# apache/arrow

Hardware: AMD Instinct MI355X
Metric: filter_take_mrows_per_s (higher is better)
Workload: dtype int64; 1 GPU; Filter+Take int64[1000000000] + validity (10% null), boolean mask 10% true, FilterOptions::DROP; take indices = the mask's row numbers (monotonic; indices_nonzero: uint64 through CallFunction, GetTakeIndices: uint32 in the mirror), no boundscheck; inputs = splitmix64 streams of SURVEY.md 8(d) (seeds 1,2,3); rows=1000000000, selected_rows=99992053, parallelism=single-gpu

## Files before the change

arrow_amd/_lib.py:

```python
from __future__ import annotations

import ctypes as C
import os

_HERE = os.path.dirname(os.path.abspath(__file__))
LIB_PATH = os.path.join(_HERE, "libarrow_amd.so")

ARX_OK = 0
ARX_OUT_OF_MEMORY = -1
ARX_INVALID = -4
ARX_CAPACITY_ERROR = -6
ARX_INDEX_ERROR = -7
ARX_NOT_IMPLEMENTED = -10
ARX_DEVICE_ERROR = -100

ABI_VERSION = 3

FILTER_DROP, FILTER_EMIT_NULL = 0, 1
SORT_ASCENDING, SORT_DESCENDING = 0, 1
NULLS_AT_START, NULLS_AT_END = 0, 1


class ArrowAmdError(Exception):
    """Base class; subclasses mirror pyarrow.lib.ArrowInvalid & friends."""
# ... 61 lines not shown
        ("validity", C.c_void_p),
        ("offsets", C.c_void_p),
        ("data", C.c_void_p),
        ("offset", C.c_int64),
        ("length", C.c_int64),
        ("null_count", C.c_int64),
    ]


_p, _i64, _int, _u64, _u32, _sz = C.c_void_p, C.c_int64, C.c_int, C.c_uint64, C.c_uint32, C.c_size_t
_span = C.POINTER(ArxSpan)
_bspan = C.POINTER(ArxBinarySpan)

SIGNATURES = {
    "arx_last_error": (C.c_char_p, []),
    "arx_abi_version": (_int, []),
    "arx_device_count": (_int, []),
    "arx_set_option": (_int, [C.c_char_p, _i64]),
    "arx_get_counter": (_i64, [C.c_char_p]),
    "arx_filter_workspace_bytes": (_sz, [_i64]),
    "arx_filter_count": (_int, [_span, _int, _p, _sz, C.POINTER(_i64), _p]),
    "arx_filter_count_async": (_int, [_span, _int, _p, _sz, _p]),
    "arx_filter_count_nulls": (_int, [_span, _span, _int, _p, _sz, C.POINTER(_i64), C.POINTER(_i64), _p]),
    "arx_filter_exec": (_int, [_span, _int, _span, _int, _p, _i64, _p, _p, _p]),
    "arx_mask_to_indices": (_int, [_span, _int, _p, _i64, _int, _p, _p, _p]),
    "arx_take_workspace_bytes": (_sz, []),
    "arx_check_index_bounds": (_int, [_span, _int, _u64, _p, _sz, _p]),
    "arx_take": (_int, [_span, _int, _span, _int, _p, _p, _p, _p]),
    "arx_take_rows": (_int, [_span, _i64, _span, _int, _p, _p, _p, _p]),
    "arx_take_bits": (_int, [_span, _span, _int, _p, _p, _p, _p]),
    "arx_binary_take_workspace_bytes": (_sz, [_i64]),
    "arx_binary_take_offsets": (_int, [_bspan, _span, _int, _p, _sz, _p, _p, _p, C.POINTER(_i64), _p]),
    "arx_binary_take_data": (_int, [_bspan, _i64, _p, _sz, _p, _i64, _p, _p]),
    "arx_large_binary_take_workspace_bytes": (_sz, [_i64]),
    "arx_large_binary_take_offsets": (_int, [_bspan, _span, _int, _p, _sz, _p, _p, _p, C.POINTER(_i64), _p]),
    "arx_large_binary_take_data": (_int, [_bspan, _i64, _p, _sz, _p, _i64, _p, _p]),
    "arx_list_take_data": (_int, [_bspan, _int, _i64, _p, _sz, _p, _i64, _p, _p]),
    "arx_large_list_take_data": (_int, [_bspan, _int, _i64, _p, _sz, _p, _i64, _p, _p]),
    "arx_plain_byte_array_offsets": (_int, [_p, _sz, _i64, C.c_int32, _p]),
    "arx_rle_scan_runs": (_int, [_p, _sz, _int, _i64, _u32, _u64, _p, _i64, C.POINTER(_i64), C.POINTER(_i64)]),
    "arx_rle_decode_u32": (_int, [_p, _sz, _p, _i64, _int, _i64, _p, _p]),
    "arx_rle_decode_equals_bitmap": (_int, [_p, _sz, _p, _i64, _int, _i64, _u32, _p, _p]),
    "arx_expand_by_mask": (_int, [_p, _int, _span, _p, _p, _p]),
    "arx_rle_levels_to_bitmap": (_int, [_p, _p, _i64, _p, _p, _p, _p]),
    "arx_rle_scan_runs_equals": (_int, [_p, _sz, _int, _i64, _u32, _u32, _u64, _p, _i64, C.POINTER(_i64), C.POINTER(_i64)]),
    "arx_levels_to_list_workspace_bytes": (_sz, [_i64]),
# ... 191 lines not shown
```

arrow_amd/csrc/plugin/common.inc:

```

std::atomic<int64_t> g_gpu_calls{0};
std::atomic<int64_t> g_stock_calls{0};
std::atomic<int64_t> g_min_rows{1 << 16};
std::atomic<int64_t> g_min_rows_streaming{INT64_MAX};
std::atomic<int64_t> g_filter_morsel_rows{[] {
  const char* env = std::getenv("ARROW_AMD_FILTER_MORSEL_ROWS");
  return env != nullptr ? static_cast<int64_t>(std::strtoll(env, nullptr, 10)) : int64_t(1) << 20;
}()};

std::atomic<bool> g_parquet_pinned_staging{true};
std::atomic<bool> g_parquet_device_levels{true};
std::atomic<int> g_parquet_read_threads{4};
std::atomic<int64_t> g_parquet_read_part_bytes{int64_t(1) << 23};
std::atomic<bool> g_parquet_device_snappy{[] {
  const char* env = std::getenv("ARROW_AMD_PARQUET_DEVICE_SNAPPY");
  return env == nullptr || std::strtoll(env, nullptr, 10) != 0;
}()};
std::atomic<int64_t> g_parquet_device_snappy_pages{0};
std::atomic<bool> g_parquet_device_gzip{true};
std::atomic<int64_t> g_parquet_device_gzip_pages{0};
std::atomic<int64_t> g_parquet_copied_pages{0};

std::atomic<int64_t> g_aggregate_flush_rows{[] {
  const char* env = std::getenv("ARROW_AMD_AGGREGATE_FLUSH_ROWS");
// ... 119 lines not shown
      ptr_ = nullptr;
      size_ = 0;
      const size_t want = std::max<size_t>(bytes + bytes / 4, size_t(1) << 20);
      HIP_RETURN_NOT_OK(hipHostMalloc(&ptr_, want, hipHostMallocDefault));
      size_ = want;
    }
    *out = static_cast<uint8_t*>(ptr_);
    return Status::OK();
  }
  void Trim(size_t keep_at_most) {
    if (size_ > keep_at_most && ptr_ != nullptr) {
      (void)hipHostFree(ptr_);
      ptr_ = nullptr;
      size_ = 0;
    }
  }

 private:
  void* ptr_ = nullptr;
  size_t size_ = 0;
};
thread_local PinnedStaging t_pinned;

enum Slot { kValues = 0, kValidity, kArg2, kArg2Validity, kOutData, kOutValidity, kWs, kCounter, kBinWs, kFlag };

Status Upload(const ArraySpan& a, int byte_width_or_0_for_bool, int data_slot, int validity_slot,
              hipStream_t st, ArxSpan* out) {
  const int64_t o8 = a.offset % 8;
  const int64_t first = a.offset - o8;
  out->offset = o8;
  out->length = a.length;
  out->null_count = a.null_count;
  out->validity = nullptr;
  out->data = nullptr;
  const int64_t span_elems = o8 + a.length;
  if (a.buffers[1].data != nullptr && a.length > 0) {
    const uint8_t* src;
    size_t bytes;
    if (byte_width_or_0_for_bool == 0) {
      src = a.buffers[1].data + first / 8;
      bytes = static_cast<size_t>(arrow::bit_util::BytesForBits(span_elems));
    } else {
      src = a.buffers[1].data + first * byte_width_or_0_for_bool;
      bytes = static_cast<size_t>(span_elems) * byte_width_or_0_for_bool;
    }
    void* d = nullptr;
// ... 66 lines not shown
```

arrow_amd/csrc/plugin/selection.inc:

```
StockKernel g_stock_filter;

arrow::Result<std::unique_ptr<cp::KernelState>> FilterInit(cp::KernelContext* ctx,
                                                           const cp::KernelInitArgs& args) {
  auto state = std::make_unique<ShimState<cp::FilterOptions>>();
  if (g_stock_filter.init) {
    ARROW_ASSIGN_OR_RAISE(state->stock, g_stock_filter.init(ctx, args));
  }
  if (args.options != nullptr) {
    state->options = *static_cast<const cp::FilterOptions*>(args.options);
  }
  return state;
}

Status BooleanTakeOnDevice(const ArxSpan& dv, const ArxSpan& di, int tid, hipStream_t st, ArrayData* out_arr) {
  const int64_t m = di.length;
  const int64_t bytes = ((m + 63) / 64) * 8;
  const bool allocate_validity = dv.null_count != 0 || di.null_count != 0;
  out_arr->length = m;
  out_arr->buffers.resize(2);
  out_arr->buffers[0] = nullptr;
  ARROW_ASSIGN_OR_RAISE(out_arr->buffers[1], AllocDevice(bytes));
  void* d_valid = nullptr;
  void* d_counter = nullptr;
  if (allocate_validity) {
// ... 108 lines not shown
        d_valid = reinterpret_cast<void*>(out_arr->buffers[0]->mutable_address());
      }
      ARROW_RETURN_NOT_OK(FromArx(arx_filter_exec(&dv, w, &dm, null_sel, ws, n,
                                                  reinterpret_cast<void*>(out_arr->buffers[1]->mutable_address()),
                                                  d_valid, st)));
      int64_t selected = 0, set_bits = 0;
      HIP_RETURN_NOT_OK(hipMemcpyAsync(&selected, ws, 8, hipMemcpyDeviceToHost, st));
      if (allocate_validity) {
        void* cws = nullptr;
        ARROW_RETURN_NOT_OK(t_scratch.Get(kCounter, 64, &cws));
        ARROW_RETURN_NOT_OK(FromArx(arx_bitmap_popcount(d_valid, 0, n, cws, 64, &set_bits, st)));
      } else {
        HIP_RETURN_NOT_OK(hipStreamSynchronize(st));
      }
      out_arr->length = selected;
      out_arr->null_count = allocate_validity ? selected - set_bits : 0;
      static_cast<RocmBuffer*>(out_arr->buffers[1].get())->Shrink(selected * w);
      if (allocate_validity) static_cast<RocmBuffer*>(out_arr->buffers[0].get())->Shrink(((selected + 63) / 64) * 8);
      CountGpu(kFnFilter);
      return Status::OK();
    }
    int64_t out_len = 0, out_nulls = 0;
    if (allocate_validity) {
      ARROW_RETURN_NOT_OK(FromArx(arx_filter_count_nulls(&dv, &dm, null_sel, ws, ws_bytes, &out_len, &out_nulls, st)));
    } else {
      ARROW_RETURN_NOT_OK(FromArx(arx_filter_count(&dm, null_sel, ws, ws_bytes, &out_len, st)));
    }
    out_arr->length = out_len;
    out_arr->buffers.resize(2);
    ARROW_ASSIGN_OR_RAISE(out_arr->buffers[1], AllocDevice(out_len * w));
    out_arr->buffers[0] = nullptr;
    void* d_valid = nullptr;
    if (allocate_validity) {
      ARROW_ASSIGN_OR_RAISE(out_arr->buffers[0], AllocDevice(((out_len + 63) / 64) * 8));
      d_valid = reinterpret_cast<void*>(out_arr->buffers[0]->mutable_address());
    }
    ARROW_RETURN_NOT_OK(FromArx(arx_filter_exec(&dv, w, &dm, null_sel, ws, out_len,
                                                reinterpret_cast<void*>(out_arr->buffers[1]->mutable_address()),
                                                d_valid, st)));
    out_arr->null_count = allocate_validity ? out_nulls : 0;
    HIP_RETURN_NOT_OK(hipStreamSynchronize(st));
    CountGpu(kFnFilter);
    return Status::OK();
  }
  if (w == 0 || filter.type->id() != Type::BOOL || values.length < g_min_rows.load() ||
      !IsHost(values) || !IsHost(filter)) {
    return RunStock(kFnFilter, g_stock_filter, state->stock.get(), ctx, batch, out);
  }
  hipStream_t st;
// ... 262 lines not shown
    if (w == 0 || tid < 0) {
      return Status::NotImplemented("arrow_amd: take of ", values.type->ToString(), " by ",
                                    indices.type->ToString(), " on device-resident arrays");
    }
    hipStream_t st;
    ARROW_RETURN_NOT_OK(t_scratch.Stream(&st));
    ArxSpan dv{}, di{};
    ARROW_RETURN_NOT_OK(DeviceSpan(values, &dv));
    ARROW_RETURN_NOT_OK(DeviceSpan(indices, &di));
    if (state->options.boundscheck) ARROW_RETURN_NOT_OK(CheckBoundsOnDevice(di, tid, values.length, st));
    const int64_t m = indices.length;
    const bool allocate_validity = dv.null_count != 0 || di.null_count != 0;
    ArrayData* out_arr = out->array_data().get();
    out_arr->length = m;
    out_arr->buffers.resize(2);
    ARROW_ASSIGN_OR_RAISE(out_arr->buffers[1], AllocDevice(m * w));
    out_arr->buffers[0] = nullptr;
    void* d_valid = nullptr;
    void* d_counter = nullptr;
    if (allocate_validity) {
      ARROW_ASSIGN_OR_RAISE(out_arr->buffers[0], AllocDevice(((m + 63) / 64) * 8));
      d_valid = reinterpret_cast<void*>(out_arr->buffers[0]->mutable_address());
      ARROW_RETURN_NOT_OK(t_scratch.Get(kCounter, 64, &d_counter));
      HIP_RETURN_NOT_OK(hipMemsetAsync(d_counter, 0, 8, st));
    }
    ARROW_RETURN_NOT_OK(FromArx(arx_take(&dv, w, &di, tid,
                                         reinterpret_cast<void*>(out_arr->buffers[1]->mutable_address()), d_valid,
                                         static_cast<int64_t*>(d_counter), st)));
    int64_t valid_count = m;
    if (allocate_validity) {
      HIP_RETURN_NOT_OK(hipMemcpyAsync(&valid_count, d_counter, 8, hipMemcpyDeviceToHost, st));
    }
    HIP_RETURN_NOT_OK(hipStreamSynchronize(st));
    out_arr->null_count = m - valid_count;
    CountGpu(kFnTake);
    return Status::OK();
  }
  if (w == 0 || tid < 0 || indices.length < g_min_rows.load() || !IsHost(values) || !IsHost(indices)) {
    return RunStock(kFnTake, g_stock_take, state->stock.get(), ctx, batch, out);
  }
  hipStream_t st;
  ARROW_RETURN_NOT_OK(t_scratch.Stream(&st));
  ArxSpan dv{}, di{};
  ARROW_RETURN_NOT_OK(Upload(values, w, kValues, kValidity, st, &dv));
  ARROW_RETURN_NOT_OK(Upload(indices, kIdxWidth[tid], kArg2, kArg2Validity, st, &di));
  if (state->options.boundscheck) ARROW_RETURN_NOT_OK(CheckBoundsOnDevice(di, tid, values.length, st));
  const int64_t m = indices.length;
  const bool allocate_validity = values.MayHaveNulls() || indices.MayHaveNulls();
  ArrayData* out_arr = out->array_data().get();
  out_arr->length = m;
  out_arr->buffers.resize(2);
  ARROW_ASSIGN_OR_RAISE(out_arr->buffers[1], ctx->Allocate(m * w));
  void* d_out = nullptr;
  void* d_out_valid = nullptr;
  void* d_counter = nullptr;
  ARROW_RETURN_NOT_OK(t_scratch.Get(kOutData, static_cast<size_t>(m) * w + 16, &d_out));
// ... 25 lines not shown
```

arrow_amd/csrc/plugin/vector_hash.inc:

```
enum HashVectorKind { kHashUnique = 0, kHashValueCounts, kHashDictEncode };

struct DeviceHashState : public cp::KernelState {
  HashVectorKind kind = kHashUnique;
  std::unique_ptr<cp::KernelState> stock;
  bool used_stock = false, used_device = false;
  bool encode_nulls = false;
  std::shared_ptr<arrow::DataType> type;
  int width = 0;
  std::shared_ptr<Buffer> table_buf, counts_buf;
  void* table = nullptr;
  int64_t max_groups = 0, num_groups = 0, counts_cap = 0;
};

StockKernel g_stock_unique, g_stock_value_counts, g_stock_dict_encode;
cp::VectorKernel::FinalizeFunc g_stock_unique_finalize = nullptr, g_stock_value_counts_finalize = nullptr,
                               g_stock_dict_encode_finalize = nullptr;

template <HashVectorKind KIND>
const StockKernel& StockHashKernel() {
  return KIND == kHashUnique ? g_stock_unique : KIND == kHashValueCounts ? g_stock_value_counts : g_stock_dict_encode;
}

void* Align256(const std::shared_ptr<Buffer>& b) {
  return reinterpret_cast<void*>((b->mutable_address() + 255) & ~uintptr_t(255));
// ... 297 lines not shown
  } else {
    const int num = NonZeroNumericTypeId(in.type->id());
    if (num < 0) return Status::NotImplemented("arrow_amd: indices_nonzero of device-resident ", in.type->ToString(), " arrays");
    static const int widths[10] = {1, 1, 2, 2, 4, 4, 8, 8, 4, 8};
    ARROW_ASSIGN_OR_RAISE(bits, AllocDevice(((n + 63) / 64) * 8 + 8));
    const uint64_t zero = 0;
    const uint8_t* base = static_cast<const uint8_t*>(dv.data) + dv.offset * widths[num];
    if (n > 0) {
      ARROW_RETURN_NOT_OK(FromArx(arx_compare_numeric(ARX_CMP_NOT_EQUAL, num, base, nullptr, nullptr, &zero, n,
                                                      reinterpret_cast<uint64_t*>(bits->mutable_address()), st)));
    }
    dm.data = reinterpret_cast<const void*>(bits->address());
    dm.offset = 0;
    if (dm.validity != nullptr && dv.offset != 0) {
      ARROW_ASSIGN_OR_RAISE(rebased, AllocDevice(((n + 63) / 64) * 8 + 8));
      ARROW_RETURN_NOT_OK(FromArx(arx_bitmap_copy(dv.validity, dv.offset, n, reinterpret_cast<void*>(rebased->mutable_address()), st)));
      dm.validity = reinterpret_cast<const void*>(rebased->address());
    }
  }
  const size_t ws_bytes = arx_filter_workspace_bytes(n);
  void* ws = nullptr;
  ARROW_RETURN_NOT_OK(t_scratch.Get(kWs, ws_bytes, &ws));
  int64_t cnt = 0;
  if (n > 0) ARROW_RETURN_NOT_OK(FromArx(arx_filter_count(&dm, ARX_FILTER_DROP, ws, ws_bytes, &cnt, st)));
  void* d_idx = nullptr;
  ARROW_RETURN_NOT_OK(t_scratch.Get(kArg2, static_cast<size_t>(cnt) * 4 + 64, &d_idx));
  ARROW_ASSIGN_OR_RAISE(auto out_values, AllocDevice(std::max<int64_t>(cnt, 1) * 8));
  bool direct = false;
  if (cnt > 0) {
    direct = arx_mask_to_indices(&dm, ARX_FILTER_DROP, ws, cnt, 8, reinterpret_cast<void*>(out_values->mutable_address()), nullptr, st) == ARX_OK;
  }
  if (cnt > 0 && !direct) {
    ARROW_RETURN_NOT_OK(FromArx(arx_mask_to_indices(&dm, ARX_FILTER_DROP, ws, cnt, 4, d_idx, nullptr, st)));
    ArxSpan di{nullptr, d_idx, 0, cnt, 0};
    void* flag = nullptr;
    ARROW_RETURN_NOT_OK(t_scratch.Get(kFlag, 64, &flag));
    ARROW_RETURN_NOT_OK(FromArx(arx_cast_numeric(&di, ARX_NUM_UINT32, ARX_NUM_UINT64, 1, 1, flag, 64,
                                                 reinterpret_cast<void*>(out_values->mutable_address()), st)));
  }
  HIP_RETURN_NOT_OK(hipStreamSynchronize(st));
  CountGpu(kFnFilter);
  out->value = ArrayData::Make(arrow::uint64(), cnt, {nullptr, std::move(out_values)}, 0);
  return Status::OK();
}

Status RegisterIndicesNonZero(cp::FunctionRegistry* reg) {
  ARROW_ASSIGN_OR_RAISE(auto fn, reg->GetFunction("indices_nonzero"));
  if (fn->kind() != cp::Function::VECTOR) return Status::Invalid("indices_nonzero is not a vector function");
  auto* vfn = static_cast<cp::VectorFunction*>(fn.get());
  for (const auto& ty : {arrow::boolean(), arrow::int8(), arrow::uint8(), arrow::int16(), arrow::uint16(), arrow::int32(),
                         arrow::uint32(), arrow::int64(), arrow::uint64(), arrow::float32(), arrow::float64()}) {
    ARROW_ASSIGN_OR_RAISE(const cp::Kernel* k0, vfn->DispatchExact({ty}));
    cp::VectorKernel copy = *static_cast<const cp::VectorKernel*>(k0);
    if (g_stock_nonzero.exec == nullptr) g_stock_nonzero.exec = copy.exec;
    if (g_stock_nonzero.exec != copy.exec) continue;
// ... 64 lines not shown
```

arrow_amd/csrc/selection.hip:

```cpp
#include "arx_common.h"

#include <string.h>

#include <algorithm>
#include <type_traits>

namespace arx {

struct FilterWsHeader {
  int64_t total;
  int64_t ntiles;
  int64_t ngroups;
  int64_t length;
  int64_t valid;
  int64_t pad[3];
};
static_assert(sizeof(FilterWsHeader) == 64, "header is one 64-byte line");

struct FilterWsView {
  FilterWsHeader* hdr;
  int64_t* group_excl;
  int64_t* group_total;
  uint32_t* tile_counts;
  int64_t* group_valid;
};

static inline int64_t num_tiles(int64_t length) { return ceil_div(length, kTileRows); }
static inline int64_t num_groups(int64_t length) {
// ... 5 lines not shown
  const int64_t ng = num_groups(length);
  uint8_t* p = static_cast<uint8_t*>(ws);
  v.hdr = reinterpret_cast<FilterWsHeader*>(p);
  v.group_excl = reinterpret_cast<int64_t*>(p + 64);
  v.group_total = v.group_excl + ng;
  v.tile_counts = reinterpret_cast<uint32_t*>(v.group_total + ng);
  v.group_valid = reinterpret_cast<int64_t*>(v.tile_counts + ng * kTilesPerGroup);
  return v;
}

__device__ __forceinline__ uint64_t emit_word(const Bits& mask, const Bits& mvalid, int64_t w,
                                              bool emit_null, bool invert,
                                              uint64_t* mask_valid_out) {
  uint64_t m = load_word(mask, w);
  const uint64_t mv = load_word(mvalid, w);
  *mask_valid_out = mv;
  if (emit_null || invert) {
    const uint64_t in_range = load_word(Bits{nullptr, 0, mask.length, 0}, w);
    if (invert) m = ~m & in_range;
    if (emit_null) return (m | ~mv) & in_range;
  }
  return m & mv;
}

template <bool VALID>
__global__ __launch_bounds__(kBlock) void count_kernel(Bits mask, Bits mvalid, Bits vvalid, int emit_null,
                                                       int invert, int64_t ntiles,
                                                       uint32_t* tile_counts,
                                                       int64_t* group_total, int64_t* group_valid) {
  __shared__ uint32_t wave_sums[kWavesPerBlock];
  __shared__ uint32_t wave_valid[kWavesPerBlock];
  const int lane = lane_id();
  const int wave = threadIdx.x >> 6;
  const int64_t group = blockIdx.x;
  const int64_t t0 = group * kTilesPerGroup + wave * 16;
  uint32_t mine = 0;
  uint32_t kv = 0;
#pragma unroll 4
  for (int i = 0; i < 16; ++i) {
    const int64_t t = t0 + i;
    uint32_t k = 0;
    if (t < ntiles) {
      uint64_t mv;
      const uint64_t e = emit_word(mask, mvalid, t * 64 + lane, emit_null != 0, invert != 0, &mv);
      k = __popcll(e);
      if constexpr (VALID) kv += __popcll(e & mv & load_word(vvalid, t * 64 + lane));
// ... 2 lines not shown
    if (lane == i) mine = s;
  }
  if (lane < 16) tile_counts[t0 + lane] = mine;
  const uint32_t wsum = wave_reduce_sum_u32(lane < 16 ? mine : 0u);
  if (lane == 0) wave_sums[wave] = wsum;
  if constexpr (VALID) {
    const uint32_t vsum = wave_reduce_sum_u32(kv);
    if (lane == 0) wave_valid[wave] = vsum;
  }
  __syncthreads();
  if (threadIdx.x == 0) {
    int64_t s = 0, v = 0;
    for (int i = 0; i < kWavesPerBlock; ++i) {
      s += wave_sums[i];
      if constexpr (VALID) v += wave_valid[i];
    }
    group_total[group] = s;
    if constexpr (VALID) group_valid[group] = v;
  }
}

__global__ __launch_bounds__(1024) void scan_kernel(const int64_t* group_total, int64_t ngroups,
                                                    int64_t* group_excl, FilterWsHeader* hdr,
                                                    const int64_t* group_valid = nullptr) {
  __shared__ int64_t wave_tot[16];
  __shared__ int64_t carry_s;
  __shared__ unsigned long long valid_s;
  const int tid = threadIdx.x;
  const int lane = tid & 63;
  const int wave = tid >> 6;
  if (tid == 0) carry_s = 0;
  if (tid == 0) valid_s = 0;
  __syncthreads();
  if (group_valid != nullptr) {
    int64_t mine = 0;
    for (int64_t i = tid; i < ngroups; i += 1024) mine += group_valid[i];
#pragma unroll
    for (int d = 32; d >= 1; d >>= 1) mine += __shfl_xor(mine, d, 64);
    if (lane == 0 && mine != 0) atomicAdd(&valid_s, static_cast<unsigned long long>(mine));
    __syncthreads();
  }
  for (int64_t base = 0; base < ngroups; base += 1024) {
    const int64_t i = base + tid;
    const int64_t v = i < ngroups ? group_total[i] : 0;
    int64_t x = v;
#pragma unroll
    for (int d = 1; d < 64; d <<= 1) {
      const int64_t n = __shfl_up(x, d, 64);
      if (lane >= d) x += n;
    }
    if (lane == 63) wave_tot[wave] = x;
    __syncthreads();
    int64_t wave_prefix = 0;
    for (int k = 0; k < wave; ++k) wave_prefix += wave_tot[k];
    const int64_t carry = carry_s;
    if (i < ngroups) group_excl[i] = carry + wave_prefix + x - v;
    __syncthreads();
    if (tid == 1023) carry_s = carry + wave_prefix + x;
    __syncthreads();
  }
  if (tid == 0) {
    hdr->total = carry_s;
    hdr->valid = static_cast<int64_t>(valid_s);
  }
}

struct CompactArgs {
  const uint8_t* values;
  Bits mask;
  Bits mvalid;
  Bits vvalid;
  int64_t length;
  int64_t ntiles;
  const uint32_t* tile_counts;
  const int64_t* group_excl;
  uint8_t* out_data;
  uint64_t* out_validity;
  int emit_null;
  int invert;
  int values_aligned16;
};

constexpr int kFlushBytes = 2048;

template <int RING>
// ... 542 lines not shown
      if (upto > done) {
        const uint64_t span = (upto - done >= 64 ? ~uint64_t(0) : ((uint64_t(1) << (upto - done)) - 1)) << done;
        if ((load_word(vsel, r >> 6) >> (r & 63)) & 1ull) bits |= span;
        if ((load_word(vvalid, r >> 6) >> (r & 63)) & 1ull) valid |= span;
        done = upto;
      }
    }
    out_bits[w] = bits;
    if (out_valid != nullptr) out_valid[w] = valid;
  }
}

struct TakeArgs {
  const uint8_t* values;
  Bits vvalid_unused;
  const uint8_t* src_valid_bytes;
  int64_t src_valid_offset;
  const uint8_t* indices;
  Bits ivalid;
  int64_t length;
  uint8_t* out_data;
  uint64_t* out_validity;
  unsigned long long* valid_count;
};

template <int W, typename IdxT, bool HAS_IV, bool HAS_SV>
__global__ __launch_bounds__(kBlock) void take_kernel(TakeArgs a) {
  using E = typename ElemT<W>::type;
  constexpr int U = 8;
  const int lane = lane_id();
  const int64_t nwaves = static_cast<int64_t>(gridDim.x) * kWavesPerBlock;
  const int64_t wave_g = static_cast<int64_t>(blockIdx.x) * kWavesPerBlock +
                         __builtin_amdgcn_readfirstlane(threadIdx.x >> 6);
  const int64_t nchunks = (a.length + 64 * U - 1) / (64 * U);
  const int64_t last = a.length - 1;
  const IdxT* __restrict__ indices = reinterpret_cast<const IdxT*>(a.indices);
  const E* __restrict__ values = reinterpret_cast<const E*>(a.values);
  E* __restrict__ out = reinterpret_cast<E*>(a.out_data);
  uint64_t nvalid = 0;
  for (int64_t c = wave_g; c < nchunks; c += nwaves) {
    const int64_t base = c * (64 * U);
    int64_t pos[U];
    uint64_t idx[U];
    bool ok[U];
#pragma unroll
    for (int u = 0; u < U; ++u) {
// ... 19 lines not shown
      uint8_t vb[U];
#pragma unroll
      for (int u = 0; u < U; ++u) {
        const uint64_t bit = ok[u] ? static_cast<uint64_t>(a.src_valid_offset) + idx[u] : 0;
        vb[u] = a.src_valid_bytes[bit >> 3];
      }
#pragma unroll
      for (int u = 0; u < U; ++u) {
        const uint64_t bit = static_cast<uint64_t>(a.src_valid_offset) + idx[u];
        ok[u] = ok[u] && ((vb[u] >> (bit & 7)) & 1);
      }
    }
#pragma unroll
    for (int u = 0; u < U; ++u) {
      const int64_t p = base + u * 64 + lane;
      if (p <= last) sel_store<W>(out + p, ok[u] ? val[u] : zero_elem<W>());
      const uint64_t vbal = __ballot(ok[u]);
      nvalid += __popcll(vbal);
      if (a.out_validity != nullptr && lane == 0 && (base + u * 64) <= last) {
        a.out_validity[(base >> 6) + u] = vbal;
      }
    }
  }
  if (a.valid_count != nullptr && lane == 0 && nvalid != 0) atomicAdd(a.valid_count, nvalid);
}

template <int UB> struct RowUnit;
template <> struct RowUnit<1> { typedef uint8_t type; };
template <> struct RowUnit<2> { typedef uint16_t type; };
template <> struct RowUnit<4> { typedef uint32_t type; };
template <> struct RowUnit<8> { typedef uint64_t type; };
template <> struct RowUnit<16> { typedef arx_u32x4 type; };

template <int UB, typename IdxT, bool HAS_IV, bool HAS_SV>
__global__ __launch_bounds__(kBlock) void take_rows_kernel(TakeArgs a, uint32_t units_per_row) {
  using E = typename RowUnit<UB>::type;
  const int lane = lane_id();
  const int64_t nwaves = static_cast<int64_t>(gridDim.x) * kWavesPerBlock;
  const int64_t wave_g = static_cast<int64_t>(blockIdx.x) * kWavesPerBlock + __builtin_amdgcn_readfirstlane(threadIdx.x >> 6);
  const int64_t nchunks = (a.length + 63) >> 6;
  const int64_t last = a.length - 1;
  const IdxT* __restrict__ indices = reinterpret_cast<const IdxT*>(a.indices);
  const E* __restrict__ values = reinterpret_cast<const E*>(a.values);
  E* __restrict__ out = reinterpret_cast<E*>(a.out_data);
  uint64_t nvalid = 0;
  for (int64_t c = wave_g; c < nchunks; c += nwaves) {
    const int64_t base = c << 6;
// ... 208 lines not shown
  if (mask == nullptr) {
    set_error("filter mask is NULL");
    return ARX_INVALID;
  }
  if (mask->length < 0 || mask->offset < 0) {
    set_error("negative length/offset");
    return ARX_INVALID;
  }
  if (mask->length > 0 && mask->data == nullptr) {
    set_error("filter mask has no data buffer");
    return ARX_INVALID;
  }
  if (null_selection != ARX_FILTER_DROP && null_selection != ARX_FILTER_EMIT_NULL) {
    set_error("bad null_selection %d", null_selection);
    return ARX_INVALID;
  }
  return ARX_OK;
}

static inline const void* effective_validity(const ArxSpan* s) {
  return (s->null_count != 0) ? s->validity : nullptr;
}

static int launch_count(const ArxSpan* mask, int null_selection, void* ws, size_t ws_bytes,
                        hipStream_t st, int invert = 0, const ArxSpan* values = nullptr) {
  const int rc = check_mask(mask, null_selection);
  if (rc != ARX_OK) return rc;
  const size_t need = arx_filter_workspace_bytes(mask->length);
  if (ws == nullptr || ws_bytes < need) {
    set_error("filter workspace too small: %zu < %zu", ws_bytes, need);
    return ARX_INVALID;
  }
  if ((reinterpret_cast<uint64_t>(ws) & 63) != 0) {
    set_error("filter workspace must be 64-byte aligned");
    return ARX_INVALID;
  }
  FilterWsView v = ws_view(ws, mask->length);
  const int64_t nt = num_tiles(mask->length);
  const int64_t ng = num_groups(mask->length);
  FilterWsHeader h{};
  h.total = 0;
  h.ntiles = nt;
  h.ngroups = ng;
  h.length = mask->length;
  ARX_HIP(hipMemcpyAsync(v.hdr, &h, sizeof(h), hipMemcpyHostToDevice, st));
  if (mask->length == 0) return ARX_OK;
  const Bits mb = make_bits(mask->data, mask->offset, mask->length);
  const Bits mvb = make_bits(effective_validity(mask), mask->offset, mask->length);
  if (values != nullptr) {
    const Bits vvb = make_bits(effective_validity(values), values->offset, mask->length);
    hipLaunchKernelGGL((count_kernel<true>), dim3(static_cast<unsigned>(ng)), dim3(kBlock), 0, st, mb, mvb, vvb,
                       null_selection, invert, nt, v.tile_counts, v.group_total, v.group_valid);
    ARX_CHECK_LAUNCH("count_kernel");
    hipLaunchKernelGGL(scan_kernel, dim3(1), dim3(1024), 0, st, v.group_total, ng, v.group_excl, v.hdr,
                       static_cast<const int64_t*>(v.group_valid));
  } else {
    hipLaunchKernelGGL((count_kernel<false>), dim3(static_cast<unsigned>(ng)), dim3(kBlock), 0, st, mb, mvb, mvb,
                       null_selection, invert, nt, v.tile_counts, v.group_total, static_cast<int64_t*>(nullptr));
    ARX_CHECK_LAUNCH("count_kernel");
    hipLaunchKernelGGL(scan_kernel, dim3(1), dim3(1024), 0, st, v.group_total, ng, v.group_excl, v.hdr,
                       static_cast<const int64_t*>(nullptr));
  }
  ARX_CHECK_LAUNCH("scan_kernel");
  return ARX_OK;
}

static Knob<int> g_filter_batch{4};
static Knob<int> g_filter_pipe{1};
static Knob<int> g_filter_sparse{-1};

template <int W, bool IOTA, bool EMIT, bool ALIGNED>
static void launch_compact_e(const CompactArgs& a, unsigned grid, hipStream_t st) {
  constexpr int kIters = kTileRows / (kWave * (16 / W));
  constexpr int kBig = kIters >= 8 ? 4 : 2;
  if (ALIGNED && g_filter_batch >= 4 && g_filter_pipe) {
    hipLaunchKernelGGL((compact_kernel<W, IOTA, EMIT, ALIGNED, kBig, true>), dim3(grid),
                       dim3(kBlock), 0, st, a);
  } else {
    hipLaunchKernelGGL((compact_kernel<W, IOTA, EMIT, ALIGNED, 1, false>), dim3(grid), dim3(kBlock),
                       0, st, a);
  }
}

template <int W, bool IOTA>
static void launch_compact_w(const CompactArgs& a, unsigned grid, hipStream_t st) {
  const bool aligned = IOTA || a.values_aligned16 != 0;
  if (a.emit_null) {
    if (aligned) launch_compact_e<W, IOTA, true, true>(a, grid, st);
// ... 53 lines not shown
  } else {
    switch (W) {
      case 1: launch_compact_w<1, false>(a, grid, st); break;
      case 2: launch_compact_w<2, false>(a, grid, st); break;
      case 4: launch_compact_w<4, false>(a, grid, st); break;
      case 8: launch_compact_w<8, false>(a, grid, st); break;
      case 16: launch_compact_w<16, false>(a, grid, st); break;
      default:
        set_error("unsupported byte width %d for the gfx950 filter", W);
        return ARX_NOT_IMPLEMENTED;
    }
  }
  ARX_CHECK_LAUNCH("compact_kernel");
  return ARX_OK;
}

int set_selection_option(const char* name, int64_t value) {
  if (strcmp(name, "filter_batch") == 0) {
    g_filter_batch = value >= 4 ? 4 : 1;
    return 1;
  }
  if (strcmp(name, "filter_pipe") == 0) {
    g_filter_pipe = value != 0;
    return 1;
  }
  if (strcmp(name, "filter_sparse") == 0) {
    g_filter_sparse = value < 0 ? -1 : (value != 0);
    return 1;
  }
  return 0;
}

static int zero_out_validity(void* out_validity, int64_t out_length, hipStream_t st) {
  if (out_validity == nullptr) return ARX_OK;
  if ((reinterpret_cast<uint64_t>(out_validity) & 7) != 0) {
    set_error("out_validity must be 8-byte aligned");
    return ARX_INVALID;
  }
  if (out_length < 0) {
    set_error("out_length (from arx_filter_count) is required when out_validity is given");
    return ARX_INVALID;
  }
  if (out_length > 0) {
    ARX_HIP(hipMemsetAsync(out_validity, 0, static_cast<size_t>(ceil_div(out_length, 64)) * 8, st));
  }
  return ARX_OK;
// ... 32 lines not shown
  a.emit_null = 0;
  a.invert = invert ? 1 : 0;
  a.values_aligned16 = 1;
  return launch_compact(true, 4, a, st);
}

}

using namespace arx;

extern "C" {

size_t arx_filter_workspace_bytes(int64_t length) {
  if (length < 0) length = 0;
  const int64_t ng = num_groups(length);
  return static_cast<size_t>(64 + ng * 16 + ng * kTilesPerGroup * 4 + ng * 8 + 64);
}

int arx_filter_count_async(const ArxSpan* mask, int null_selection, void* ws, size_t ws_bytes,
                           void* stream) {
  return launch_count(mask, null_selection, ws, ws_bytes, as_stream(stream));
}

int arx_filter_count_nulls(const ArxSpan* values, const ArxSpan* mask, int null_selection, void* ws, size_t ws_bytes,
                           int64_t* out_length, int64_t* out_null_count, void* stream) {
  if (out_length == nullptr || out_null_count == nullptr || values == nullptr) {
    set_error("values / out_length / out_null_count is NULL");
    return ARX_INVALID;
  }
  if (mask != nullptr && values->length != mask->length) {
    set_error("filter values and mask differ in length (%lld vs %lld)", static_cast<long long>(values->length),
              static_cast<long long>(mask->length));
    return ARX_INVALID;
  }
  hipStream_t st = as_stream(stream);
  const int rc = launch_count(mask, null_selection, ws, ws_bytes, st, 0, values);
  if (rc != ARX_OK) return rc;
  int64_t hdr[5] = {0, 0, 0, 0, 0};
  ARX_HIP(hipMemcpyAsync(hdr, ws, sizeof(hdr), hipMemcpyDeviceToHost, st));
  ARX_HIP(hipStreamSynchronize(st));
  *out_length = hdr[0];
  *out_null_count = mask->length == 0 ? 0 : hdr[0] - hdr[4];
  return ARX_OK;
}

int arx_filter_count(const ArxSpan* mask, int null_selection, void* ws, size_t ws_bytes,
                     int64_t* out_length, void* stream) {
  if (out_length == nullptr) {
    set_error("out_length is NULL");
    return ARX_INVALID;
  }
  hipStream_t st = as_stream(stream);
  const int rc = launch_count(mask, null_selection, ws, ws_bytes, st);
  if (rc != ARX_OK) return rc;
  int64_t total = 0;
  ARX_HIP(hipMemcpyAsync(&total, ws, sizeof(int64_t), hipMemcpyDeviceToHost, st));
  ARX_HIP(hipStreamSynchronize(st));
  *out_length = total;
  return ARX_OK;
}

int arx_filter_exec(const ArxSpan* values, int byte_width, const ArxSpan* mask, int null_selection,
                    const void* ws, int64_t out_length, void* out_data, void* out_validity,
                    void* stream) {
  int rc = check_mask(mask, null_selection);
// ... 175 lines not shown
  ARX_HIP(hipStreamSynchronize(st));
  if (res.first_bad_pos != ~0ull) {
    const bool is_signed = (index_type & 1) != 0;
    if (is_signed) {
      set_error("Index %lld out of bounds", res.bad_value_signed);
    } else {
      set_error("Index %llu out of bounds", res.bad_value_unsigned);
    }
    return ARX_INDEX_ERROR;
  }
  return ARX_OK;
}

int arx_take(const ArxSpan* values, int byte_width, const ArxSpan* indices, int index_type,
             void* out_data, void* out_validity, int64_t* valid_count, void* stream) {
  if (values == nullptr || indices == nullptr) {
    set_error("values/indices is NULL");
    return ARX_INVALID;
  }
  if (index_type < 0 || index_type > 7) {
    set_error("Unsupported index type %d for take", index_type);
    return ARX_NOT_IMPLEMENTED;
  }
  if (indices->length == 0) return ARX_OK;
  if (out_data == nullptr || indices->data == nullptr) {
    set_error("indices/out data buffer is NULL");
    return ARX_INVALID;
  }
  static const int widths[8] = {1, 1, 2, 2, 4, 4, 8, 8};
  const int iw = widths[index_type];
  hipStream_t st = as_stream(stream);
  TakeArgs a{};
  a.values = static_cast<const uint8_t*>(values->data) + values->offset * byte_width;
  a.src_valid_bytes = static_cast<const uint8_t*>(effective_validity(values));
  a.src_valid_offset = values->offset;
  a.indices = static_cast<const uint8_t*>(indices->data) + indices->offset * iw;
  a.ivalid = make_bits(effective_validity(indices), indices->offset, indices->length);
  a.length = indices->length;
  a.out_data = static_cast<uint8_t*>(out_data);
  a.out_validity = static_cast<uint64_t*>(out_validity);
  a.valid_count = reinterpret_cast<unsigned long long*>(valid_count);
  const bool needs_validity = a.src_valid_bytes != nullptr || a.ivalid.base != nullptr;
  if (needs_validity && out_validity == nullptr) {
    set_error("take: inputs may have nulls but out_validity is NULL");
    return ARX_INVALID;
  }
  const int64_t nchunks = ceil_div(indices->length, 512);
  const int64_t blocks = std::min<int64_t>(ceil_div(nchunks, kWavesPerBlock), 256 * 32);
  const dim3 grid(static_cast<unsigned>(blocks)), block(kBlock);
  const bool has_iv = a.ivalid.base != nullptr;
  const bool has_sv = a.src_valid_bytes != nullptr;
#define ARX_TAKE_V(WW, IT)                                                                     \
  do {                                                                                         \
    if (has_iv && has_sv) hipLaunchKernelGGL((take_kernel<WW, IT, true, true>), grid, block, 0, st, a);        \
    else if (has_iv) hipLaunchKernelGGL((take_kernel<WW, IT, true, false>), grid, block, 0, st, a);            \
    else if (has_sv) hipLaunchKernelGGL((take_kernel<WW, IT, false, true>), grid, block, 0, st, a);            \
    else hipLaunchKernelGGL((take_kernel<WW, IT, false, false>), grid, block, 0, st, a);                       \
  } while (0)
#define ARX_TAKE_W(WW)                      \
  switch (iw) {                             \
    case 1: ARX_TAKE_V(WW, uint8_t); break; \
    case 2: ARX_TAKE_V(WW, uint16_t); break;\
    case 4: ARX_TAKE_V(WW, uint32_t); break;\
    default: ARX_TAKE_V(WW, uint64_t); break;\
  }
  switch (byte_width) {
    case 1: ARX_TAKE_W(1); break;
    case 2: ARX_TAKE_W(2); break;
// ... 235 lines not shown
```

include/arrow_amd.h:

```cpp
#ifndef ARROW_AMD_H_
#define ARROW_AMD_H_

#include <stddef.h>
#include <stdint.h>

#ifdef __cplusplus
extern "C" {
#endif

#define ARX_ABI_VERSION 3

typedef enum ArxStatus {
  ARX_OK = 0,
  ARX_OUT_OF_MEMORY = -1,
  ARX_INVALID = -4,
  ARX_CAPACITY_ERROR = -6,
  ARX_INDEX_ERROR = -7,
  ARX_NOT_IMPLEMENTED = -10,
  ARX_DEVICE_ERROR = -100
} ArxStatus;

enum { ARX_FILTER_DROP = 0, ARX_FILTER_EMIT_NULL = 1 };
enum { ARX_SORT_ASCENDING = 0, ARX_SORT_DESCENDING = 1 };
enum { ARX_NULLS_AT_START = 0, ARX_NULLS_AT_END = 1 };
// ... 8 lines not shown
  const void* data;
  int64_t offset;
  int64_t length;
  int64_t null_count;
} ArxSpan;

const char* arx_last_error(void);
int arx_abi_version(void);
int arx_device_count(void);
int arx_set_option(const char* name, int64_t value);
int64_t arx_get_counter(const char* name);


size_t arx_filter_workspace_bytes(int64_t length);

int arx_filter_count(const ArxSpan* mask, int null_selection, void* ws, size_t ws_bytes,
                     int64_t* out_length, void* stream);

int arx_filter_count_nulls(const ArxSpan* values, const ArxSpan* mask, int null_selection, void* ws, size_t ws_bytes,
                           int64_t* out_length, int64_t* out_null_count, void* stream);

int arx_filter_count_async(const ArxSpan* mask, int null_selection, void* ws,
                           size_t ws_bytes, void* stream);

int arx_filter_exec(const ArxSpan* values, int byte_width, const ArxSpan* mask,
                    int null_selection, const void* ws, int64_t out_length, void* out_data,
                    void* out_validity, void* stream);

int arx_mask_to_indices(const ArxSpan* mask, int null_selection, const void* ws,
                        int64_t out_length, int index_width, void* out_indices,
                        void* out_validity, void* stream);

size_t arx_take_workspace_bytes(void);

int arx_check_index_bounds(const ArxSpan* indices, int index_type, uint64_t upper_limit,
                           void* ws, size_t ws_bytes, void* stream);

int arx_take(const ArxSpan* values, int byte_width, const ArxSpan* indices, int index_type,
             void* out_data, void* out_validity, int64_t* valid_count, void* stream);

int arx_take_rows(const ArxSpan* values, int64_t row_bytes, const ArxSpan* indices, int index_type, void* out_data,
                  void* out_validity, int64_t* valid_count, void* stream);

int arx_take_columns(const ArxSpan* columns, const int32_t* byte_widths, int num_columns, const ArxSpan* indices,
                     int index_type, void* const* out_data, void* const* out_validity, int64_t* valid_counts,
                     void* stream);
// ... 500 lines not shown
```

Baseline: 308,500 Mrows/s.

## Cut host-device round trips in filter count and take null counting

Moves the filter workspace header fill from a host-to-device memcpy into the scan kernel, and reads count results back through a thread-local pinned buffer instead of pageable memory. The take kernel now counts valid rows through a per-thread device arrival slot: the last wave to arrive writes the final count and resets the slot, which removes the memset before each take. A new async count-with-nulls entry point is added. These changes target small fixed per-call costs (memcpy, memset, pageable sync), so any gain on a billion-row workload will be small. The per-thread slot pool adds correctness risk if two streams on the same thread run takes at once.

Measured after the change: 311,700 Mrows/s, median of 6. +1.0%, better.

```diff
diff --git a/arrow_amd/_lib.py b/arrow_amd/_lib.py
--- a/arrow_amd/_lib.py
+++ b/arrow_amd/_lib.py
@@ -107,6 +107,7 @@
     "arx_filter_count": (_int, [_span, _int, _p, _sz, C.POINTER(_i64), _p]),
     "arx_filter_count_async": (_int, [_span, _int, _p, _sz, _p]),
     "arx_filter_count_nulls": (_int, [_span, _span, _int, _p, _sz, C.POINTER(_i64), C.POINTER(_i64), _p]),
+    "arx_filter_count_nulls_async": (_int, [_span, _span, _int, _p, _sz, _p]),
     "arx_filter_exec": (_int, [_span, _int, _span, _int, _p, _i64, _p, _p, _p]),
     "arx_mask_to_indices": (_int, [_span, _int, _p, _i64, _int, _p, _p, _p]),
     "arx_take_workspace_bytes": (_sz, []),
diff --git a/arrow_amd/csrc/plugin/common.inc b/arrow_amd/csrc/plugin/common.inc
--- a/arrow_amd/csrc/plugin/common.inc
+++ b/arrow_amd/csrc/plugin/common.inc
@@ -165,6 +165,26 @@
 };
 thread_local PinnedStaging t_pinned;
 
+class PinnedReadback {
+ public:
+  ~PinnedReadback() {
+    if (ptr_) (void)hipHostFree(ptr_);
+  }
+  Status ReadBack(const void* d_src, int n, hipStream_t st, int64_t* out) {
+    if (!ptr_) HIP_RETURN_NOT_OK(hipHostMalloc(&ptr_, kWords * sizeof(int64_t), hipHostMallocDefault));
+    if (n < 0 || n > kWords) return Status::Invalid("arrow_amd: read-back of ", n, " words");
+    HIP_RETURN_NOT_OK(hipMemcpyAsync(ptr_, d_src, static_cast<size_t>(n) * sizeof(int64_t), hipMemcpyDeviceToHost, st));
+    HIP_RETURN_NOT_OK(hipStreamSynchronize(st));
+    std::memcpy(out, ptr_, static_cast<size_t>(n) * sizeof(int64_t));
+    return Status::OK();
+  }
+
+ private:
+  static constexpr int kWords = 8;
+  void* ptr_ = nullptr;
+};
+thread_local PinnedReadback t_readback;
+
 enum Slot { kValues = 0, kValidity, kArg2, kArg2Validity, kOutData, kOutValidity, kWs, kCounter, kBinWs, kFlag };
 
 Status Upload(const ArraySpan& a, int byte_width_or_0_for_bool, int data_slot, int validity_slot,
diff --git a/arrow_amd/csrc/plugin/selection.inc b/arrow_amd/csrc/plugin/selection.inc
--- a/arrow_amd/csrc/plugin/selection.inc
+++ b/arrow_amd/csrc/plugin/selection.inc
@@ -154,9 +154,14 @@
     }
     int64_t out_len = 0, out_nulls = 0;
     if (allocate_validity) {
-      ARROW_RETURN_NOT_OK(FromArx(arx_filter_count_nulls(&dv, &dm, null_sel, ws, ws_bytes, &out_len, &out_nulls, st)));
+      ARROW_RETURN_NOT_OK(FromArx(arx_filter_count_nulls_async(&dv, &dm, null_sel, ws, ws_bytes, st)));
+      int64_t hdr[5];
+      ARROW_RETURN_NOT_OK(t_readback.ReadBack(ws, 5, st, hdr));
+      out_len = hdr[0];
+      out_nulls = hdr[0] - hdr[4];
     } else {
-      ARROW_RETURN_NOT_OK(FromArx(arx_filter_count(&dm, null_sel, ws, ws_bytes, &out_len, st)));
+      ARROW_RETURN_NOT_OK(FromArx(arx_filter_count_async(&dm, null_sel, ws, ws_bytes, st)));
+      ARROW_RETURN_NOT_OK(t_readback.ReadBack(ws, 1, st, &out_len));
     }
     out_arr->length = out_len;
     out_arr->buffers.resize(2);
@@ -465,16 +470,16 @@
       ARROW_ASSIGN_OR_RAISE(out_arr->buffers[0], AllocDevice(((m + 63) / 64) * 8));
       d_valid = reinterpret_cast<void*>(out_arr->buffers[0]->mutable_address());
       ARROW_RETURN_NOT_OK(t_scratch.Get(kCounter, 64, &d_counter));
-      HIP_RETURN_NOT_OK(hipMemsetAsync(d_counter, 0, 8, st));
     }
     ARROW_RETURN_NOT_OK(FromArx(arx_take(&dv, w, &di, tid,
                                          reinterpret_cast<void*>(out_arr->buffers[1]->mutable_address()), d_valid,
                                          static_cast<int64_t*>(d_counter), st)));
     int64_t valid_count = m;
     if (allocate_validity) {
-      HIP_RETURN_NOT_OK(hipMemcpyAsync(&valid_count, d_counter, 8, hipMemcpyDeviceToHost, st));
-    }
-    HIP_RETURN_NOT_OK(hipStreamSynchronize(st));
+      ARROW_RETURN_NOT_OK(t_readback.ReadBack(d_counter, 1, st, &valid_count));
+    } else {
+      HIP_RETURN_NOT_OK(hipStreamSynchronize(st));
+    }
     out_arr->null_count = m - valid_count;
     CountGpu(kFnTake);
     return Status::OK();
diff --git a/arrow_amd/csrc/plugin/vector_hash.inc b/arrow_amd/csrc/plugin/vector_hash.inc
--- a/arrow_amd/csrc/plugin/vector_hash.inc
+++ b/arrow_amd/csrc/plugin/vector_hash.inc
@@ -343,15 +343,18 @@
   void* ws = nullptr;
   ARROW_RETURN_NOT_OK(t_scratch.Get(kWs, ws_bytes, &ws));
   int64_t cnt = 0;
-  if (n > 0) ARROW_RETURN_NOT_OK(FromArx(arx_filter_count(&dm, ARX_FILTER_DROP, ws, ws_bytes, &cnt, st)));
-  void* d_idx = nullptr;
-  ARROW_RETURN_NOT_OK(t_scratch.Get(kArg2, static_cast<size_t>(cnt) * 4 + 64, &d_idx));
+  if (n > 0) {
+    ARROW_RETURN_NOT_OK(FromArx(arx_filter_count_async(&dm, ARX_FILTER_DROP, ws, ws_bytes, st)));
+    ARROW_RETURN_NOT_OK(t_readback.ReadBack(ws, 1, st, &cnt));
+  }
   ARROW_ASSIGN_OR_RAISE(auto out_values, AllocDevice(std::max<int64_t>(cnt, 1) * 8));
   bool direct = false;
   if (cnt > 0) {
     direct = arx_mask_to_indices(&dm, ARX_FILTER_DROP, ws, cnt, 8, reinterpret_cast<void*>(out_values->mutable_address()), nullptr, st) == ARX_OK;
   }
   if (cnt > 0 && !direct) {
+    void* d_idx = nullptr;
+    ARROW_RETURN_NOT_OK(t_scratch.Get(kArg2, static_cast<size_t>(cnt) * 4 + 64, &d_idx));
     ARROW_RETURN_NOT_OK(FromArx(arx_mask_to_indices(&dm, ARX_FILTER_DROP, ws, cnt, 4, d_idx, nullptr, st)));
     ArxSpan di{nullptr, d_idx, 0, cnt, 0};
     void* flag = nullptr;
diff --git a/arrow_amd/csrc/selection.hip b/arrow_amd/csrc/selection.hip
--- a/arrow_amd/csrc/selection.hip
+++ b/arrow_amd/csrc/selection.hip
@@ -3,7 +3,9 @@
 #include <string.h>
 
 #include <algorithm>
+#include <mutex>
 #include <type_traits>
+#include <vector>
 
 namespace arx {
 
@@ -55,6 +57,10 @@
   }
   return m & mv;
 }
+
+constexpr int kArrivalSlots = 1024;
+constexpr int kTakeCountBits = 40;
+__device__ unsigned long long g_take_count[kArrivalSlots];
 
 template <bool VALID>
 __global__ __launch_bounds__(kBlock) void count_kernel(Bits mask, Bits mvalid, Bits vvalid, int emit_null,
@@ -103,7 +109,7 @@
 
 __global__ __launch_bounds__(1024) void scan_kernel(const int64_t* group_total, int64_t ngroups,
                                                     int64_t* group_excl, FilterWsHeader* hdr,
-                                                    const int64_t* group_valid = nullptr) {
+                                                    const int64_t* group_valid, int64_t ntiles, int64_t length) {
   __shared__ int64_t wave_tot[16];
   __shared__ int64_t carry_s;
   __shared__ unsigned long long valid_s;
@@ -142,6 +148,9 @@
   }
   if (tid == 0) {
     hdr->total = carry_s;
+    hdr->ntiles = ntiles;
+    hdr->ngroups = ngroups;
+    hdr->length = length;
     hdr->valid = static_cast<int64_t>(valid_s);
   }
 }
@@ -730,6 +739,7 @@
   uint8_t* out_data;
   uint64_t* out_validity;
   unsigned long long* valid_count;
+  int slot;
 };
 
 template <int W, typename IdxT, bool HAS_IV, bool HAS_SV>
@@ -795,7 +805,16 @@
       }
     }
   }
-  if (a.valid_count != nullptr && lane == 0 && nvalid != 0) atomicAdd(a.valid_count, nvalid);
+  if (a.valid_count == nullptr || lane != 0) return;
+  if (a.slot < 0) {
+    if (nvalid != 0) atomicAdd(a.valid_count, nvalid);
+    return;
+  }
+  const unsigned long long mine = (1ull << kTakeCountBits) + static_cast<unsigned long long>(nvalid);
+  const unsigned long long before = atomicAdd(&g_take_count[a.slot], mine);
+  if ((before >> kTakeCountBits) != static_cast<unsigned long long>(nwaves) - 1) return;
+  atomicExch(&g_take_count[a.slot], 0ull);
+  *a.valid_count = (before & ((1ull << kTakeCountBits) - 1)) + static_cast<unsigned long long>(nvalid);
 }
 
 template <int UB> struct RowUnit;
@@ -1050,6 +1069,34 @@
   return (s->null_count != 0) ? s->validity : nullptr;
 }
 
+static int thread_arrival_slot() {
+  struct Pool {
+    std::mutex mu;
+    std::vector<int> free;
+    int next = 0;
+  };
+  static Pool* pool = new Pool();
+  struct Owner {
+    int id = -2;
+    ~Owner() {
+      if (id < 0) return;
+      std::lock_guard<std::mutex> lock(pool->mu);
+      pool->free.push_back(id);
+    }
+  };
+  thread_local Owner owner;
+  if (owner.id == -2) {
+    std::lock_guard<std::mutex> lock(pool->mu);
+    if (!pool->free.empty()) {
+      owner.id = pool->free.back();
+      pool->free.pop_back();
+    } else {
+      owner.id = pool->next < kArrivalSlots ? pool->next++ : -1;
+    }
+  }
+  return owner.id;
+}
+
 static int launch_count(const ArxSpan* mask, int null_selection, void* ws, size_t ws_bytes,
                         hipStream_t st, int invert = 0, const ArxSpan* values = nullptr) {
   const int rc = check_mask(mask, null_selection);
@@ -1066,13 +1113,10 @@
   FilterWsView v = ws_view(ws, mask->length);
   const int64_t nt = num_tiles(mask->length);
   const int64_t ng = num_groups(mask->length);
-  FilterWsHeader h{};
-  h.total = 0;
-  h.ntiles = nt;
-  h.ngroups = ng;
-  h.length = mask->length;
-  ARX_HIP(hipMemcpyAsync(v.hdr, &h, sizeof(h), hipMemcpyHostToDevice, st));
-  if (mask->length == 0) return ARX_OK;
+  if (mask->length == 0) {
+    ARX_HIP(hipMemsetAsync(v.hdr, 0, sizeof(FilterWsHeader), st));
+    return ARX_OK;
+  }
   const Bits mb = make_bits(mask->data, mask->offset, mask->length);
   const Bits mvb = make_bits(effective_validity(mask), mask->offset, mask->length);
   if (values != nullptr) {
@@ -1081,17 +1125,19 @@
                        null_selection, invert, nt, v.tile_counts, v.group_total, v.group_valid);
     ARX_CHECK_LAUNCH("count_kernel");
     hipLaunchKernelGGL(scan_kernel, dim3(1), dim3(1024), 0, st, v.group_total, ng, v.group_excl, v.hdr,
-                       static_cast<const int64_t*>(v.group_valid));
+                       static_cast<const int64_t*>(v.group_valid), nt, mask->length);
   } else {
     hipLaunchKernelGGL((count_kernel<false>), dim3(static_cast<unsigned>(ng)), dim3(kBlock), 0, st, mb, mvb, mvb,
                        null_selection, invert, nt, v.tile_counts, v.group_total, static_cast<int64_t*>(nullptr));
     ARX_CHECK_LAUNCH("count_kernel");
     hipLaunchKernelGGL(scan_kernel, dim3(1), dim3(1024), 0, st, v.group_total, ng, v.group_excl, v.hdr,
-                       static_cast<const int64_t*>(nullptr));
+                       static_cast<const int64_t*>(nullptr), nt, mask->length);
   }
   ARX_CHECK_LAUNCH("scan_kernel");
   return ARX_OK;
 }
+
+static Knob<int> g_take_count_fused{1};
 
 static Knob<int> g_filter_batch{4};
 static Knob<int> g_filter_pipe{1};
@@ -1191,6 +1237,10 @@
   }
   if (strcmp(name, "filter_pipe") == 0) {
     g_filter_pipe = value != 0;
+    return 1;
+  }
+  if (strcmp(name, "take_count_fused") == 0) {
+    g_take_count_fused = value != 0;
     return 1;
   }
   if (strcmp(name, "filter_sparse") == 0) {
@@ -1269,10 +1319,10 @@
   return launch_count(mask, null_selection, ws, ws_bytes, as_stream(stream));
 }
 
-int arx_filter_count_nulls(const ArxSpan* values, const ArxSpan* mask, int null_selection, void* ws, size_t ws_bytes,
-                           int64_t* out_length, int64_t* out_null_count, void* stream) {
-  if (out_length == nullptr || out_null_count == nullptr || values == nullptr) {
-    set_error("values / out_length / out_null_count is NULL");
+int arx_filter_count_nulls_async(const ArxSpan* values, const ArxSpan* mask, int null_selection, void* ws,
+                                 size_t ws_bytes, void* stream) {
+  if (values == nullptr) {
+    set_error("values is NULL");
     return ARX_INVALID;
   }
   if (mask != nullptr && values->length != mask->length) {
@@ -1280,14 +1330,23 @@
               static_cast<long long>(mask->length));
     return ARX_INVALID;
   }
+  return launch_count(mask, null_selection, ws, ws_bytes, as_stream(stream), 0, values);
+}
+
+int arx_filter_count_nulls(const ArxSpan* values, const ArxSpan* mask, int null_selection, void* ws, size_t ws_bytes,
+                           int64_t* out_length, int64_t* out_null_count, void* stream) {
+  if (out_length == nullptr || out_null_count == nullptr) {
+    set_error("values / out_length / out_null_count is NULL");
+    return ARX_INVALID;
+  }
   hipStream_t st = as_stream(stream);
-  const int rc = launch_count(mask, null_selection, ws, ws_bytes, st, 0, values);
+  const int rc = arx_filter_count_nulls_async(values, mask, null_selection, ws, ws_bytes, stream);
   if (rc != ARX_OK) return rc;
   int64_t hdr[5] = {0, 0, 0, 0, 0};
   ARX_HIP(hipMemcpyAsync(hdr, ws, sizeof(hdr), hipMemcpyDeviceToHost, st));
   ARX_HIP(hipStreamSynchronize(st));
   *out_length = hdr[0];
-  *out_null_count = mask->length == 0 ? 0 : hdr[0] - hdr[4];
+  *out_null_count = hdr[0] - hdr[4];
   return ARX_OK;
 }
 
@@ -1509,7 +1568,10 @@
     set_error("Unsupported index type %d for take", index_type);
     return ARX_NOT_IMPLEMENTED;
   }
-  if (indices->length == 0) return ARX_OK;
+  if (indices->length == 0) {
+    if (valid_count != nullptr) ARX_HIP(hipMemsetAsync(valid_count, 0, sizeof(int64_t), as_stream(stream)));
+    return ARX_OK;
+  }
   if (out_data == nullptr || indices->data == nullptr) {
     set_error("indices/out data buffer is NULL");
     return ARX_INVALID;
@@ -1527,10 +1589,15 @@
   a.out_data = static_cast<uint8_t*>(out_data);
   a.out_validity = static_cast<uint64_t*>(out_validity);
   a.valid_count = reinterpret_cast<unsigned long long*>(valid_count);
+  a.slot = -1;
   const bool needs_validity = a.src_valid_bytes != nullptr || a.ivalid.base != nullptr;
   if (needs_validity && out_validity == nullptr) {
     set_error("take: inputs may have nulls but out_validity is NULL");
     return ARX_INVALID;
+  }
+  if (valid_count != nullptr) {
+    a.slot = g_take_count_fused && indices->length < (int64_t(1) << kTakeCountBits) ? thread_arrival_slot() : -1;
+    if (a.slot < 0) ARX_HIP(hipMemsetAsync(valid_count, 0, sizeof(int64_t), st));
   }
   const int64_t nchunks = ceil_div(indices->length, 512);
   const int64_t blocks = std::min<int64_t>(ceil_div(nchunks, kWavesPerBlock), 256 * 32);
diff --git a/include/arrow_amd.h b/include/arrow_amd.h
--- a/include/arrow_amd.h
+++ b/include/arrow_amd.h
@@ -54,6 +54,8 @@
 
 int arx_filter_count_async(const ArxSpan* mask, int null_selection, void* ws,
                            size_t ws_bytes, void* stream);
+int arx_filter_count_nulls_async(const ArxSpan* values, const ArxSpan* mask, int null_selection, void* ws,
+                                 size_t ws_bytes, void* stream);
 
 int arx_filter_exec(const ArxSpan* values, int byte_width, const ArxSpan* mask,
                     int null_selection, const void* ws, int64_t out_length, void* out_data,
```
